# dbking77/ar_slam

Hardware: AMD Instinct MI355X
Metric: LM iterations/sec + ms-to-converged reproj-RMS, 10k-capture synthetic graph (higher is better)
Workload: dtype f64

## Files before the change

ar_slam_amd/build.py:

```python
from __future__ import annotations

import os
import shutil
import subprocess
import sys

HERE = os.path.dirname(os.path.abspath(__file__))
ROOT = os.path.dirname(HERE)
CSRC = os.path.join(HERE, "csrc")
LIB = os.environ.get("ARSLAM_LIB") or os.path.join(HERE, "libarslam_lm.so")
SOURCES = ["lm_kernels.hip", "dense_llt.hip", "lm_solver.hip", "debug_api.hip", "llt_plan.cpp",
           "host_structure.cpp", "localize.hip"]
HOST = os.path.join(HERE, "host")
HOST_SOURCES = ["yaml_lite.cpp", "ar_slam_solver.cpp", "slam_capi.cpp"]
ARCH = os.environ.get("ARSLAM_ARCH", "gfx950")


def hipcc():
    for cand in (shutil.which("hipcc"), "/opt/rocm/bin/hipcc"):
        if cand and os.path.exists(cand):
            return cand
    raise RuntimeError("hipcc not found")


# ... 14 lines not shown
        fcntl.flock(lock, fcntl.LOCK_EX)
        if not force and not _stale():
            return LIB
        return _build_locked(verbose)


def build_id():
    import hashlib
    h = hashlib.sha256(os.environ.get("ARSLAM_EXTRA_FLAGS", "").encode())
    files = [os.path.join(CSRC, f) for f in SOURCES] + [os.path.join(HOST, f) for f in HOST_SOURCES] + \
        sorted(os.path.join(d, f) for d in (CSRC, HOST, os.path.join(ROOT, "include"))
               for f in os.listdir(d) if f.endswith((".h", ".hpp")))
    for f in files:
        with open(f, "rb") as fh:
            h.update(os.path.relpath(f, ROOT).encode() + b"\0" + fh.read())
    commit = "nogit"
    try:
        commit = subprocess.run(["git", "-C", ROOT, "rev-parse", "--short=12", "HEAD"], capture_output=True,
                                text=True, timeout=10).stdout.strip() or "nogit"
        if commit != "nogit":
            rel = [os.path.relpath(f, ROOT) for f in files]
            dirty = subprocess.run(["git", "-C", ROOT, "status", "--porcelain", "--"] + rel, capture_output=True,
                                   text=True, timeout=10).stdout.strip()
            commit += "+dirty" if dirty else ""
    except (OSError, subprocess.SubprocessError):
        pass
    return f"{commit} src {h.hexdigest()[:12]}"


def _build_locked(verbose):
    extra = os.environ.get("ARSLAM_EXTRA_FLAGS", "")
    objdir = os.path.join(HERE, "_obj" + ("_" + "".join(c for c in extra if c.isalnum()) if extra else ""))
    os.makedirs(objdir, exist_ok=True)
    flags = ["-O3", f"--offload-arch={ARCH}", "-fPIC", "-std=c++17", "-munsafe-fp-atomics",
             "-Wall", "-Wno-unused-function", "-I", os.path.join(ROOT, "include"), "-I", CSRC,
             f'-DARSLAM_BUILD_ID="{build_id()}"'] + os.environ.get("ARSLAM_EXTRA_FLAGS", "").split()
    objs = []
    procs = []
    for src in SOURCES:
        obj = os.path.join(objdir, os.path.splitext(src)[0] + ".o")
        cmd = [hipcc()] + flags + (["-x", "hip"] if src.endswith(".cpp") else []) + ["-c", os.path.join(CSRC, src), "-o", obj]
        if verbose:
            print(" ".join(cmd))
        procs.append((src, subprocess.Popen(cmd, stdout=subprocess.PIPE, stderr=subprocess.STDOUT)))
        objs.append(obj)
    for src in HOST_SOURCES:
        obj = os.path.join(objdir, "host_" + os.path.splitext(src)[0] + ".o")
        cmd = ["g++", "-O2", "-fPIC", "-std=c++17", "-Wall", "-I", os.path.join(ROOT, "include"), "-I", CSRC,
               "-I", HOST, "-c", os.path.join(HOST, src), "-o", obj]
        if verbose:
            print(" ".join(cmd))
        procs.append((src, subprocess.Popen(cmd, stdout=subprocess.PIPE, stderr=subprocess.STDOUT)))
        objs.append(obj)
    errs = []
    for src, p in procs:
        out, _ = p.communicate()
        if p.returncode != 0:
            errs.append(f"--- {src} ---\n{out.decode()}")
        elif verbose and out:
            print(out.decode())
    if errs:
        raise RuntimeError("hipcc failed:\n" + "\n".join(errs))
    tmp = f"{LIB}.tmp{os.getpid()}"
    cmd = [hipcc(), f"--offload-arch={ARCH}", "-shared", "-o", tmp] + objs + \
          ["-L/opt/rocm/lib", "-lrccl", "-Wl,-rpath,/opt/rocm/lib"]
    subprocess.check_call(cmd)
    os.replace(tmp, LIB)
# ... 7 lines not shown
```

ar_slam_amd/csrc/debug_api.hip:

```cpp
#include <chrono>
#include "lm_internal.h"
#include "arslam_lm.h"
#include "arslam_lm_debug.h"

#include <climits>
#include <cstdlib>
#include <cstdio>
#include <unistd.h>
#include <cstring>
#include <string>
#include <vector>

namespace arslam {
void debug_read_schur_stamps(unsigned long long *out);
void debug_residual_jacobian(int n, const double *cam, const double *cap, const double *tag,
                             const double *corners, double *r, double *J, hipStream_t s);
void debug_angle_axis(int n, const double *w, const double *p, double *out, int *branch, hipStream_t s);
}

namespace {
int hip_fail(hipError_t e) { return e == hipSuccess ? ARSLAM_OK : ARSLAM_E_HIP; }
}

#define DBG_CHECK(x)                 \
  do {                               \
    hipError_t _e = (x);             \
    if (_e != hipSuccess) return hip_fail(_e); \
  } while (0)

extern "C" int arslam_debug_residual_jacobian(int n, const double *cam, const double *cap,
                                              const double *tag, const double *corners, double *r,
                                              double *J) {
  if (n < 0 || (n && (!cam || !cap || !tag || !corners || !r || !J))) return ARSLAM_E_INVALID_ARG;
  if (n == 0) return ARSLAM_OK;
// ... 373 lines not shown
    return ARSLAM_E_INVALID_ARG;
  }
}

extern "C" int arslam_debug_mixed_groups(const arslam_soa_problem *p, int out[4], unsigned char *e_cap,
                                         unsigned char *e_tag) {
  if (!p || !out) return ARSLAM_E_INVALID_ARG;
  try {
    std::vector<uint8_t> ec, et;
    (void)arslam::ceres_schur_side(p, &ec, &et);
    if (e_cap) std::copy(ec.begin(), ec.end(), e_cap);
    if (e_tag) std::copy(et.begin(), et.end(), e_tag);
    const arslam::MixedProblem m = arslam::mixed_problem(*p, ec, et);
    arslam::HostProblem h = arslam::host_problem(&m.soa, nullptr);
    arslam::mixed_patch(h, m, *p);
    out[0] = h.nc;
    out[1] = h.nt;
    out[2] = m.n_direct;
    out[3] = h.maxblk;
    return ARSLAM_OK;
  } catch (const arslam::ApiError &e) {
    return e.code;
  } catch (...) {
    return ARSLAM_E_INVALID_ARG;
  }
}

extern "C" int arslam_debug_schur_stamps(unsigned long long out[16]) {
  if (!out) return ARSLAM_E_INVALID_ARG;
  arslam::debug_read_schur_stamps(out);
  return ARSLAM_OK;
}

extern "C" int arslam_debug_gather_extend(const arslam_soa_problem *p, int c0, int *identical, int *n_dest) {
  if (!p || !identical || !n_dest || c0 < 0 || c0 > p->n_cap) return ARSLAM_E_INVALID_ARG;
  try {
    std::vector<int> oc, ot;
    std::vector<double> cr;
    for (int b = 0; b < p->n_obs; ++b)
      if (p->obs_cap[b] < c0) {
        oc.push_back(p->obs_cap[b]);
        ot.push_back(p->obs_tag[b]);
        cr.insert(cr.end(), p->corners + 8L * b, p->corners + 8L * b + 8);
      }
    arslam_soa_problem q = *p;
    q.n_cap = c0;
    q.n_obs = (int)oc.size();
    q.obs_cap = oc.data();
    q.obs_tag = ot.data();
    q.corners = cr.data();
    const arslam::HostProblem hs = arslam::host_problem(&q, nullptr);
    const arslam::ReducedLayout L = arslam::reduced_layout(hs, 2, true, nullptr, nullptr);
    arslam::SchurGather G = arslam::schur_gather_plan(hs, L);
    const arslam::HostProblem hf = arslam::host_problem(p, nullptr);
    arslam::schur_gather_extend(G, hf, L, c0);
    const arslam::SchurGather F = arslam::schur_gather_plan(hf, L);
    bool same = G.cap_off == F.cap_off && G.dest_row == F.dest_row && G.dest_start == F.dest_start &&
                G.items == F.items && G.splits == F.splits && G.n_pslots == F.n_pslots &&
                G.max_contrib == F.max_contrib && G.contrib.size() == F.contrib.size();
    for (size_t i = 0; same && i < G.contrib.size(); ++i)
      same = !std::memcmp(&G.contrib[i], &F.contrib[i], sizeof(arslam::SchurContrib));
    *identical = same ? 1 : 0;
    *n_dest = (int)F.dest_start.size() - 1;
    return ARSLAM_OK;
  } catch (const arslam::ApiError &e) {
    return e.code;
// ... 113 lines not shown
```

ar_slam_amd/csrc/host_structure.h:

```cpp
#pragma once

#include "arslam_lm.h"

#include <cstdint>
#include <functional>
#include <stdexcept>
#include <string>
#include <vector>

namespace arslam {

constexpr int kTileRows = 64;
constexpr int kMaxSchurBlocks = 256;

struct ApiError : std::runtime_error {
  int code;
  ApiError(int c, const std::string &m) : std::runtime_error(m), code(c) {}
};

void set_last_error(const std::string &msg);

inline void api_check(bool ok, int code, const char *msg) {
  if (!ok) throw ApiError(code, msg);
}
// ... 57 lines not shown

struct ReducedLayout {
  std::vector<int> tag_row;
  std::vector<int> row_slot;
  int cam_row = -1;
  long nR = 0, N = 0;
  int T = 0;
  std::vector<uint8_t> pattern;
  int n_parts = 0;
  long pad_rows = 0;
  double scalar_flops = 0.0;
  long n_edges = 0;
  long order_edges = 0;
  bool order_reused = false;
};

double scalar_cholesky_flops(const std::vector<std::vector<int>> &adj, const std::vector<int> &tag_row,
                             bool camera);

ReducedLayout reduced_layout(const HostProblem &h, int ordering, bool sparse, const ReduceMaxU8 &adj_max,
                             const ReduceMaxU8 &pattern_max,
                             const std::vector<int> *reuse_tag_row = nullptr, long reuse_edges = 0,
                             bool fast_order = false, bool reuse_by_identity = false);

#if defined(__HIPCC__)
#define ARSLAM_HD __host__ __device__
#else
#define ARSLAM_HD
#endif
struct SchurContrib {
  long off;
  int tr, ld;
};
ARSLAM_HD inline int schur_blk(int x, int m) { return x == 0 ? 0 : (x == m ? 1 + (m - 1) / 6 : 1 + (x - 1) / 6); }
ARSLAM_HD inline int schur_blk_size(int U, int nblk) { return (U == 0 || U == nblk + 1) ? 1 : 6; }
ARSLAM_HD inline int schur_blk_start(int U, int nblk) { return U == 0 ? 0 : (U <= nblk ? 1 + 6 * (U - 1) : 1 + 6 * nblk); }
ARSLAM_HD inline long schur_block_off(int U, int V, int nblk) {
  const long R = U == 0 ? 0 : 1 + 6L * (U - 1) + 18L * U * (U - 1);
  return R + (long)schur_blk_size(U, nblk) * schur_blk_start(V, nblk);
}
ARSLAM_HD inline long schur_slab_size(int nblk) { return 3 + 12L * nblk + 18L * nblk * (nblk + 1); }
constexpr int kSchurChunk = 64;
struct SchurGather {
  std::vector<long> cap_off;
  std::vector<int> dest_row;
  std::vector<int> dest_start;
  std::vector<SchurContrib> contrib;
  std::vector<int> items;
  std::vector<int> splits;
  int n_pslots = 0;
  int max_contrib = 0;
};
SchurGather schur_gather_plan(const HostProblem &h, const ReducedLayout &L);
void schur_gather_extend(SchurGather &G, const HostProblem &h, const ReducedLayout &L, int c0);

}
```

ar_slam_amd/csrc/lm_internal.h:

```cpp
#pragma once
#include <hip/hip_runtime.h>
#include <climits>
#include <cstdint>
#include <stdexcept>
#include <vector>

#include "host_structure.h"

namespace arslam {
constexpr int kCuFlags = 2048;
constexpr int kDagOffTicket0 = 0;
constexpr int kDagOffInflight = 1;
constexpr int kDagOffCuFlags = 2;
constexpr int kDagOffTicket1 = 2 + kCuFlags;
constexpr int kDagOffFault = 3 + kCuFlags;
enum DagFaultField {
  kFaultTicket = 0,
  kFaultKind = 1,
  kFaultCounter = 2,
  kFaultSeen = 3,
  kFaultNeed = 4,
  kFaultDrawn = 5,
  kFaultInflight = 6,
  kFaultBlock = 7,
  kFaultFirstStuck = 8,
  kDagFaultSlots = 9
};
constexpr int kDagOffStarted0 = kDagOffFault + kDagFaultSlots;
constexpr int kDagOffStarted1 = kDagOffStarted0 + 1;
constexpr int kDagCounterExtra = kDagOffStarted1 + 1;
constexpr int kDagWorkgroupsPerCu = 2;

constexpr int kWave = 64;
constexpr int kTile = 64;
constexpr int kRowStride = 14;
constexpr int kJStored = 11;
__host__ __device__ constexpr int jrow_col(int j) {
  return j <= 6 ? j : j <= 9 ? j - 6 : j <= 12 ? j - 3 : 10;
}
constexpr int kObsChunk = 8;
constexpr int kSchurMfmaBlocks = 10;
constexpr size_t schur_lds_bytes(int nblk) {
  return sizeof(double) * (6 * ((6 * nblk + 2) < 64 ? (6 * nblk + 2) : 64) + 6 * kObsChunk + 36 + 36 + 8 +
                           7 * (6 * nblk + 1) + 2 + 28 * nblk) +
         sizeof(int) * (kObsChunk + 2) + 2 * sizeof(double) + 64;
}
static_assert(schur_lds_bytes(kMaxSchurBlocks) <= 160 * 1024, "k_schur's LDS at kMaxSchurBlocks");

enum PartIdx {
  P_COST = 0,
  P_FIXED = 1,
  P_GF = 2,
  P_CF = 3,
  P_MODEL = 4,
  P_STEP2 = 5,
  P_YBAD = 6,
  P_CBAD = 7,
  NPART = 8
};

struct DevProblem {
  int nc, nt, nb;
  long n;
  long nR;
  long N;
  long lda;
  int max_obs_per_cap;
  int max_blk_per_cap;
  const int *big_caps = nullptr;
  int n_big_caps = 0;
  const int *chunk_caps = nullptr;
  int n_chunk_caps = 0;
  int swap_roles;
  const unsigned char *cap_kind = nullptr;
  const int *f_alias = nullptr;
  int nf;
  const int *fslot_row;
  int cam_row;
  const int *cap_start;
  const int *obs_tag;
// ... 266 lines not shown
```

ar_slam_amd/csrc/lm_kernels.hip:

```cpp
#include "lm_internal.h"
#include "projection.h"

#include <cfloat>
#include <mutex>
#include <string>
#include <vector>

#include "arslam_lm.h"
#include <cmath>

namespace arslam {

#ifdef ARSLAM_SCHUR_STAMPS
__device__ unsigned long long g_schur_ph[16];
#define SCHUR_STAMP_INIT unsigned long long _st0 = clock64()
#define SCHUR_STAMP(k)                                                         \
  do {                                                                         \
    const unsigned long long _n = clock64();                                   \
    if (threadIdx.x == 0) atomicAdd(&g_schur_ph[k], _n - _st0);                \
    _st0 = _n;                                                                 \
  } while (0)
void debug_read_schur_stamps(unsigned long long *out) {
  (void)hipMemcpyFromSymbol(out, HIP_SYMBOL(g_schur_ph), sizeof(g_schur_ph));
}
#else
#define SCHUR_STAMP_INIT do {} while (0)
#define SCHUR_STAMP(k) do {} while (0)
void debug_read_schur_stamps(unsigned long long *out) {
  for (int i = 0; i < 16; ++i) out[i] = 0;
}
#endif

namespace {


__device__ __forceinline__ long slot_cap(const DevProblem &P, int c) { return 3 + 6L * c; }
__device__ __forceinline__ long slot_tag(const DevProblem &P, int t) { return 3 + 6L * P.nc + 6L * t; }

__device__ __forceinline__ bool group_swapped(const DevProblem &P, int c) {
  return P.cap_kind ? P.cap_kind[c] == kMixTag : P.swap_roles != 0;
}
__device__ __forceinline__ bool group_direct(const DevProblem &P, int c) {
  return P.cap_kind && P.cap_kind[c] == kMixDirect;
}

__device__ __forceinline__ double lm_d2(const double *diag, long slot, double radius) {
  const double d = sqrt(diag[slot] / radius);
  return d * d;
}

__device__ __forceinline__ void fill_rows(const DevProblem &P, const double *x, const double *scale, int c,
                          int o0, int row0, int nr, int nrows, double *rows, double *gout = nullptr) {
  const double *cam = x;
  const double *cap = x + slot_cap(P, c);
  for (int lr = threadIdx.x; lr < nr; lr += kWave) {
    const int row = row0 + lr;
    const int q = row >> 3, corner = (row >> 1) & 3, comp = row & 1;
    const int obs = o0 + q;
    const int t = P.obs_tag[obs];
    const double *tag = x + slot_tag(P, t);
    double J[13];
    const bool sw = group_swapped(P, c);
    const double r = residual_jacobian_row(cam, sw ? tag : cap, sw ? cap : tag, corner, comp,
                                           P.corners[8L * obs + 2 * corner + comp], J);
    if (sw) {
#pragma unroll
      for (int j = 1; j < 7; ++j) {
// ... 298 lines not shown
        v = kb == 2 ? U[6 * ia + ib] : Etr[ia];
      }
      const int V = schur_blk(q, m), q0V = schur_blk_start(V, nblk);
      dst[(long)sU * q0V + ip * schur_blk_size(V, nblk) + (q - q0V)] = v;
    }
  }
}

template <bool kBig>
__global__ __launch_bounds__(kWave) void k_schur(DevProblem P, const double *__restrict__ scale,
                                                 const double *__restrict__ diag, double radius,
                                                 double *__restrict__ zero_tiles, long n_zero, ExecReset er,
                                                 const int *__restrict__ cap_list) {
  extern __shared__ __attribute__((aligned(16))) double sm[];
  SCHUR_STAMP_INIT;
  const int c = kBig ? cap_list[blockIdx.x] : (int)blockIdx.x, lane = threadIdx.x;
  if (c >= P.nc + n_zero) {
    exec_reset_elem(er, (long)(c - P.nc - n_zero) * kWave + lane);
    return;
  }
  if (c >= P.nc) {
    typedef double d2 __attribute__((ext_vector_type(2)));
    d2 *z = reinterpret_cast<d2 *>(zero_tiles + (long)(c - P.nc) * 4096);
#pragma unroll 8
    for (int e = lane; e < 2048; e += kWave) z[e] = d2{0.0, 0.0};
    return;
  }
  const int o0 = P.cap_start[c], k = P.cap_start[c + 1] - o0;
  if (k == 0) return;
  const int nrows = 8 * k;
  const int b0 = P.cap_blk_start[c], nblk = P.cap_blk_start[c + 1] - b0;
  if (!kBig && nblk > kSchurMfmaBlocks) return;
  const int m = 1 + 6 * nblk;
  double *stage = sm;
  double *tscale = stage + 6 * min(m + 1, kWave);
  double *U = tscale + 6 * kObsChunk;
  double *Ui = U + 36;
  double *Etr = Ui + 36;
  double *W = Etr + 8;
  double *Ftr = W + 6 * m;
  double *FF = Ftr + m + (m & 1);
  int *lblk = (int *)(FF + 28 * nblk);
  double *ff00 = reinterpret_cast<double *>(lblk + kObsChunk);

  const int li = lane & 15, lk = lane >> 4;
  const bool valid = li < 14;
  const double *jb = P.jrows + 8L * o0 * kJStored + (long)jrow_col(min(li, 13)) * nrows;
  double jv[16];
#pragma unroll
  for (int u = 0; u < 8; ++u)
#pragma unroll
    for (int st = 0; st < 2; ++st)
      jv[2 * u + st] = (valid && u < k) ? jb[8 * u + 4 * st + lk] : 0.0;
  static_assert(kObsChunk == 8, "k_schur's operand registers hold eight observations");
  auto stage_chunk = [&](int q0) {
    const int kc = min(kObsChunk, k - q0);
    if (lane < kc) lblk[lane] = P.obs_lblk[o0 + q0 + lane];
    if (lane < 6 * kc) tscale[lane] = scale[slot_tag(P, P.obs_tag[o0 + q0 + lane / 6]) + lane % 6];
  };
  stage_chunk(0);
  __syncthreads();
  SCHUR_STAMP(0);
  {
    for (int e = lane; e < 6 * m + m + (m & 1) + 28 * nblk; e += kWave) W[e] = 0.0;
    __builtin_amdgcn_fence(__ATOMIC_RELEASE, "wavefront");
    __builtin_amdgcn_wave_barrier();
    __builtin_amdgcn_fence(__ATOMIC_ACQUIRE, "wavefront");
    typedef double dbl4v __attribute__((ext_vector_type(4)));
    dbl4v tot = {0, 0, 0, 0};
    const double *sc = scale + slot_cap(P, c);
    const double cs = li == 0 ? scale[0] : li <= 6 ? sc[li - 1] : 1.0;
    const bool tagcol = li >= 7 && li <= 12;
    int acc_off[4], acc_stride[4];
    const int w_base = (int)(W - sm);
    {
      const int c = li, ftr0 = 6 * m, ff0 = ftr0 + m + (m & 1);
// ... 113 lines not shown
        double v = ev[i];
#pragma unroll
        for (int p = i + 1; p < 6; ++p) v -= LI6(p, i) * ev[p];
        ev[i] = v * rd[i];
      }
#pragma unroll
      for (int i = 0; i < 6; ++i) Ui[6 * i + lane] = ev[i];
    }
#undef LI6
  }
  __syncthreads();
  if (lane < 36) P.cap_ui[36L * c + lane] = Ui[lane];
  SCHUR_STAMP(2);
  SCHUR_STAMP(3);
  double *out = P.slab + P.cap_off[c];
  auto make_z = [&](int q, double z[6]) {
    if (q < m) {
      double wq[6];
#pragma unroll
      for (int b = 0; b < 6; ++b) wq[b] = W[b * m + q];
#pragma unroll
      for (int a = 0; a < 6; ++a) {
        double s = 0.0;
#pragma unroll
        for (int b = 0; b < 6; ++b) s += Ui[6 * a + b] * wq[b];
        z[a] = s;
      }
    } else {
#pragma unroll
      for (int a = 0; a < 6; ++a) z[a] = 0.0;
    }
  };
  const bool one_chunk = !kBig;
  double z[6];
  if (one_chunk) make_z(lane, z);
  if (one_chunk) {
    const int M = m + 1;
    const int li = lane & 15, lk = lane >> 4;
    double *Zs = stage;
    if (lane < M)
#pragma unroll
      for (int a = 0; a < 6; ++a) Zs[a * M + lane] = z[a];
    __builtin_amdgcn_fence(__ATOMIC_RELEASE, "wavefront");
    __builtin_amdgcn_wave_barrier();
    __builtin_amdgcn_fence(__ATOMIC_ACQUIRE, "wavefront");
    double Aop[4][2], Bop[4][2];
#pragma unroll
    for (int r = 0; r < 4; ++r)
#pragma unroll
      for (int kb = 0; kb < 2; ++kb) {
        const int a = 4 * kb + lk, pq = 16 * r + li;
        const bool in = a < 6 && pq < M;
        Aop[r][kb] = in ? (pq < m ? W[a * m + pq] : Etr[a]) : 0.0;
        Bop[r][kb] = in ? Zs[a * M + pq] : 0.0;
      }
    typedef double dbl4v __attribute__((ext_vector_type(4)));
#pragma unroll
    for (int r = 0; r < 4; ++r) {
      if (16 * r >= M) break;
      int pU[4], pI[4], pEnd[4];
      long pOff[4];
#pragma unroll
      for (int reg = 0; reg < 4; ++reg) {
        const int pp = 16 * r + lk + 4 * reg;
        const int up = pp >= 1 && pp < m ? (pp - 1) / 6 : -1;
        const int U = pp == 0 ? 0 : (pp < m ? 1 + up : nblk + 1);
        pU[reg] = U;
        pI[reg] = up >= 0 ? pp - 1 - 6 * up : 0;
        pEnd[reg] = pp == 0 ? 1 : (pp < m ? 7 + 6 * up : M);
        pOff[reg] = schur_block_off(U, 0, nblk);
      }
#pragma unroll
      for (int cc = 0; cc < 4; ++cc) {
        if (cc > r + 1 || 16 * cc >= M) break;
        dbl4v acc = {0, 0, 0, 0};
        acc = __builtin_amdgcn_mfma_f64_16x16x4f64(Aop[r][0], Bop[cc][0], acc, 0, 0, 0);
        acc = __builtin_amdgcn_mfma_f64_16x16x4f64(Aop[r][1], Bop[cc][1], acc, 0, 0, 0);
        const int q = 16 * cc + li;
        const int uq = q >= 1 && q < m ? (q - 1) / 6 : -1;
        const int V = q == 0 ? 0 : (q < m ? 1 + uq : nblk + 1);
        const int sV = schur_blk_size(V, nblk), q0V = schur_blk_start(V, nblk);
#pragma unroll
        for (int reg = 0; reg < 4; ++reg) {
          const int pp = 16 * r + lk + 4 * reg;
          if (pp >= M || q >= pEnd[reg]) continue;
          const int U = pU[reg], sU = schur_blk_size(U, nblk);
          double ff = 0.0;
          if (pp == 0) {
            ff = *ff00;
          } else if (pp == m) {
            ff = q < m ? Ftr[q] : 0.0;
          } else {
            const int up = U - 1, i = pI[reg];
            if (q == 0) {
              ff = FF[28 * up + 21 + i];
            } else if (uq == up) {
              const int iq = q - 1 - 6 * uq, lo = min(i, iq), hi = max(i, iq);
              ff = FF[28 * up + lo * 6 - lo * (lo - 1) / 2 + (hi - lo)];
            }
          }
          out[pOff[reg] + (long)sU * q0V + pI[reg] * sV + (q - q0V)] = ff - acc[reg];
        }
      }
    }
  } else
  for (int U = 0; U <= nblk + 1; ++U) {
    const int sU = schur_blk_size(U, nblk), p0U = schur_blk_start(U, nblk), ncol = p0U + sU;
    double *dst = out + schur_block_off(U, 0, nblk);
    for (int q0 = 0; q0 < ncol; q0 += kWave) {
      const int q = q0 + lane;
      if (!one_chunk) make_z(q, z);
      const int V = schur_blk(min(q, m), m), sV = schur_blk_size(V, nblk), q0V = schur_blk_start(V, nblk);
      const int uq = V - 1, iq = q - q0V;
      if (sU == 6) {
        const int up = U - 1;
        double wv[6][6];
#pragma unroll
        for (int i = 0; i < 6; ++i)
#pragma unroll
          for (int a = 0; a < 6; ++a) wv[i][a] = W[a * m + p0U + i];
#pragma unroll
        for (int i = 0; i < 6; ++i) {
          double s = 0.0;
#pragma unroll
          for (int a = 0; a < 6; ++a) s += wv[i][a] * z[a];
          double ff = 0.0;
          if (q == 0) {
            ff = FF[28 * up + 21 + i];
          } else if (uq == up) {
            const int lo = min(i, iq), hi = max(i, iq);
            ff = FF[28 * up + lo * 6 - lo * (lo - 1) / 2 + (hi - lo)];
          }
          if (q < ncol) dst[6 * q0V + i * sV + (q - q0V)] = ff - s;
        }
      } else {
// ... 857 lines not shown
```

ar_slam_amd/lm.py:

```python
from __future__ import annotations

import ctypes as C
import os

import numpy as np

HERE = os.path.dirname(os.path.abspath(__file__))
LIB_PATH = os.environ.get("ARSLAM_LIB") or os.path.join(HERE, "libarslam_lm.so")
MAX_ITERS = 1024
COMM_ID_BYTES = 128

TERMINATION = {0: "CONVERGENCE", 1: "NO_CONVERGENCE", 2: "FAILURE", 3: "USER_SUCCESS", 4: "USER_FAILURE"}
RULES = {0: "none", 1: "gradient_tolerance", 2: "parameter_tolerance", 3: "function_tolerance",
         4: "min_trust_region_radius", 5: "max_num_iterations", 6: "invalid_steps",
         7: "evaluation_failed", 8: "user_callback"}
ERRORS = {-1: "INVALID_ARG", -2: "UNSUPPORTED", -3: "NO_DEVICE", -4: "HIP", -5: "OUT_OF_MEMORY",
          -6: "COMM", -7: "STATE", -8: "DEVICE"}

EXPORTS = ["arslam_lm_options_init", "arslam_lm_create", "arslam_lm_destroy",
           "arslam_lm_set_options", "arslam_lm_get_options",
           "arslam_lm_add_residual_block", "arslam_lm_set_parameter_block_constant",
           "arslam_lm_set_parameter_block_variable", "arslam_lm_solve", "arslam_lm_reset",
           "arslam_lm_num_residual_blocks", "arslam_lm_load_soa", "arslam_lm_solve_loaded",
           "arslam_lm_solve_soa", "arslam_comm_unique_id", "arslam_lm_set_comm", "arslam_lm_set_comm_callback",
           "arslam_device_count", "arslam_lm_last_error", "arslam_lm_version",
           "arslam_lm_set_iteration_callback", "arslam_lm_owned_captures",
           "arslam_debug_residual_jacobian", "arslam_debug_dense_llt", "arslam_debug_dense_llt_ex",
           "arslam_debug_angle_axis_rotate", "arslam_lm_debug_force_indefinite",
           "arslam_lm_debug_force_multirank", "arslam_lm_debug_break_dependency", "arslam_lm_debug_tag_pair_tile",
           "arslam_debug_reduced_plan", "arslam_debug_reduced_plan_side", "arslam_debug_schur_stamps", "arslam_debug_ceres_e_blocks",
           "arslam_debug_mixed_groups",
           "arslam_debug_dag_simulate", "arslam_debug_dag_simulate_started", "arslam_debug_dag_workgroup_limit",
           "arslam_debug_dag_fault_detail", "arslam_debug_box_fingerprint",
           "arslam_debug_rank_split", "arslam_debug_gather_extend",
           "arslam_localize_many", "arslam_localizer_create", "arslam_localizer_destroy",
           "arslam_localizer_load", "arslam_localizer_solve",
           "arslam_slam_create", "arslam_slam_destroy", "arslam_slam_set_verbose", "arslam_slam_load_yaml",
           "arslam_slam_load_yaml_string", "arslam_slam_save_yaml", "arslam_slam_add_detections",
           "arslam_slam_solve", "arslam_slam_solve_incremental", "arslam_slam_localize_many",
           "arslam_slam_num_captures", "arslam_slam_num_arucos", "arslam_slam_num_blocks",
           "arslam_slam_num_solves", "arslam_slam_last_summary", "arslam_slam_solve_summary",
           "arslam_slam_solve_capture", "arslam_slam_unsolved_captures", "arslam_slam_capture", "arslam_slam_set_capture_pose", "arslam_slam_aruco", "arslam_slam_set_aruco_pose",
           "arslam_slam_block", "arslam_slam_camera", "arslam_slam_set_camera",
           "arslam_slam_get_transforms", "arslam_slam_camera_info"]

_dp = C.POINTER(C.c_double)
ALLREDUCE_FN = C.CFUNCTYPE(C.c_int, C.c_void_p, C.c_void_p, C.c_size_t, C.c_int, C.c_int)
SOLVER_CONTINUE, SOLVER_ABORT, SOLVER_TERMINATE_SUCCESSFULLY = 0, 1, 2
ELIM_AUTO, ELIM_CAPTURES, ELIM_TAGS, ELIM_MIXED = 0, 1, 2, 3
SETUP_LOAD, SETUP_VALUES, SETUP_APPEND = 0, 1, 2
_ip = C.POINTER(C.c_int)
_up = C.POINTER(C.c_ubyte)


class LMError(RuntimeError):
    def __init__(self, code, msg):
        super().__init__(f"arslam_lm error {code} ({ERRORS.get(code, '?')}): {msg}")
        self.code = code


class Options(C.Structure):
    _fields_ = [("max_num_iterations", C.c_int),
                ("function_tolerance", C.c_double), ("gradient_tolerance", C.c_double),
                ("parameter_tolerance", C.c_double),
                ("initial_trust_region_radius", C.c_double),
                ("max_trust_region_radius", C.c_double),
                ("min_trust_region_radius", C.c_double),
# ... 112 lines not shown
    L.arslam_localizer_destroy.argtypes = [C.c_void_p]
    L.arslam_localizer_destroy.restype = None
    L.arslam_localizer_load.argtypes = [C.c_void_p, C.POINTER(LocalizeBatchC)]
    L.arslam_localizer_solve.argtypes = [C.c_void_p, _dp, C.POINTER(LocalizeResult), C.POINTER(C.c_double)]
    L.arslam_lm_get_options.argtypes = [C.c_void_p, C.POINTER(Options)]
    L.arslam_lm_destroy.argtypes = [C.c_void_p]
    L.arslam_lm_destroy.restype = None
    L.arslam_lm_add_residual_block.argtypes = [C.c_void_p, _dp, _dp, _dp, _dp]
    L.arslam_lm_set_parameter_block_constant.argtypes = [C.c_void_p, _dp]
    L.arslam_lm_set_parameter_block_variable.argtypes = [C.c_void_p, _dp]
    L.arslam_lm_solve.argtypes = [C.c_void_p, C.POINTER(Summary)]
    L.arslam_lm_reset.argtypes = [C.c_void_p]
    L.arslam_lm_num_residual_blocks.argtypes = [C.c_void_p]
    L.arslam_lm_load_soa.argtypes = [C.c_void_p, C.POINTER(SoaProblem)]
    L.arslam_lm_solve_loaded.argtypes = [C.c_void_p, C.POINTER(Summary)]
    L.arslam_lm_solve_soa.argtypes = [C.POINTER(SoaProblem), C.POINTER(Options), C.POINTER(Summary)]
    L.arslam_comm_unique_id.argtypes = [C.c_char_p]
    L.arslam_lm_set_comm.argtypes = [C.c_void_p, C.c_int, C.c_int, C.c_char_p]
    L.arslam_device_count.argtypes = []
    L.arslam_lm_last_error.restype = C.c_char_p
    L.arslam_lm_version.restype = C.c_char_p
    L.arslam_debug_residual_jacobian.argtypes = [C.c_int, _dp, _dp, _dp, _dp, _dp, _dp]
    L.arslam_debug_dense_llt.argtypes = [C.c_long, _dp, _dp, _dp, C.POINTER(C.c_int)]
    L.arslam_debug_angle_axis_rotate.argtypes = [C.c_int, _dp, _dp, _dp, _ip]
    L.arslam_debug_ceres_e_blocks.argtypes = [C.POINTER(SoaProblem), _ip]
    L.arslam_debug_mixed_groups.argtypes = [C.POINTER(SoaProblem), _ip, C.POINTER(C.c_ubyte), C.POINTER(C.c_ubyte)]
    L.arslam_lm_debug_force_indefinite.argtypes = [C.c_void_p, C.c_ulonglong]
    L.arslam_lm_debug_force_multirank.argtypes = [C.c_void_p, C.c_int]
    L.arslam_debug_dag_workgroup_limit.argtypes = [C.c_int]
    L.arslam_lm_set_iteration_callback.argtypes = [C.c_void_p, ITER_CB, C.c_void_p]
    L.arslam_lm_debug_break_dependency.argtypes = [C.c_void_p, C.c_long, C.POINTER(C.c_long)]
    if hasattr(L, "arslam_lm_debug_tag_pair_tile"):
        L.arslam_lm_debug_tag_pair_tile.argtypes = [C.c_void_p, _dp, _dp, C.POINTER(C.c_int)]
    _lib = L
    return L


def _check(rc):
    if rc != 0:
        raise LMError(rc, lib().arslam_lm_last_error().decode(errors="replace"))


def device_count():
    return lib().arslam_device_count()


def make_options(**kw):
    o = Options()
    lib().arslam_lm_options_init(C.byref(o))
    for k, v in kw.items():
        if not hasattr(o, k):
            raise AttributeError(f"unknown solver option {k}")
        setattr(o, k, v)
    return o


def _f64(a, shape=None):
    a = np.ascontiguousarray(a, dtype=np.float64)
    return a if shape is None else a.reshape(shape)


class _Soa:
    def __init__(self, camera, cap, tag, obs_cap, obs_tag, corners, camera_const=False,
                 cap_const=None, tag_const=None):
        self.camera = _f64(camera).copy()
        self.cap = _f64(cap, (-1, 6)).copy()
# ... 264 lines not shown


def debug_dag_simulate(g, n_workers, seed=1, policy=0, started=None):
    A = _Soa(g.camera, g.cap, g.tag, g.obs_cap, g.obs_tag, g.corners)
    ok = C.c_int(-1)
    if started is None:
        _check(lib().arslam_debug_dag_simulate(C.byref(A.s), int(n_workers), C.c_uint(seed), int(policy),
                                               C.byref(ok)))
    else:
        _check(lib().arslam_debug_dag_simulate_started(C.byref(A.s), int(n_workers), int(started), C.c_uint(seed),
                                                       int(policy), C.byref(ok)))
    return bool(ok.value)


def debug_dag_workgroup_limit(k):
    _check(lib().arslam_debug_dag_workgroup_limit(int(k)))


def debug_dag_fault_detail(g, rec):
    A = _Soa(g.camera, g.cap, g.tag, g.obs_cap, g.obs_tag, g.corners)
    r = (C.c_int * 9)(*([int(v) for v in rec] + [0] * (9 - len(rec))))
    buf = C.create_string_buffer(4096)
    _check(lib().arslam_debug_dag_fault_detail(C.byref(A.s), r, buf, len(buf)))
    return buf.value.decode()


def debug_gather_extend(camera, cap, tag, obs_cap, obs_tag, corners, c0):
    A = _Soa(camera, cap, tag, obs_cap, obs_tag, corners)
    same, nd = C.c_int(0), C.c_int(0)
    _check(lib().arslam_debug_gather_extend(C.byref(A.s), c0, C.byref(same), C.byref(nd)))
    return bool(same.value), nd.value


class SplitInfo(C.Structure):
    _fields_ = [("tiles_per_side", C.c_int), ("n_top_cols", C.c_int), ("n_own_cols", C.c_int),
                ("n_top_tiles", C.c_long), ("n_tiles", C.c_long), ("n_dag_tasks", C.c_long),
                ("phase_split", C.c_long), ("dag_valid", C.c_int), ("n_owned_captures", C.c_int),
                ("top_work", C.c_double), ("max_rank_work", C.c_double), ("total_work", C.c_double),
                ("n_active", C.c_int)]


def debug_rank_split(camera, cap, tag, obs_cap, obs_tag, corners, nranks, rank):
    A = _Soa(camera, cap, tag, obs_cap, obs_tag, corners)
    info = SplitInfo()
    owner = np.zeros(max(A.cap.shape[0], 1), np.int32)
    _check(lib().arslam_debug_rank_split(C.byref(A.s), nranks, rank, C.byref(info), owner.ctypes.data_as(_ip)))
    return {f: getattr(info, f) for f, _ in SplitInfo._fields_}, owner[:A.cap.shape[0]]


def debug_ceres_e_blocks(camera, cap, tag, obs_cap, obs_tag, corners=None, camera_const=False, cap_const=None,
                         tag_const=None):
    if corners is None:
        corners = np.zeros((len(obs_cap), 8))
    A = _Soa(camera, cap, tag, obs_cap, obs_tag, corners, camera_const, cap_const, tag_const)
    out = np.zeros(4, np.int32)
    _check(lib().arslam_debug_ceres_e_blocks(C.byref(A.s), out.ctypes.data_as(_ip)))
    return dict(captures=int(out[0]), tags=int(out[1]), camera=int(out[2]), max_tag_obs=int(out[3]))


def debug_mixed_groups(camera, cap, tag, obs_cap, obs_tag, corners=None, camera_const=False, cap_const=None,
                       tag_const=None):
    if corners is None:
        corners = np.zeros((len(obs_cap), 8))
    A = _Soa(camera, cap, tag, obs_cap, obs_tag, corners, camera_const, cap_const, tag_const)
    out = np.zeros(4, np.int32)
    e_cap = np.zeros(max(A.cap.shape[0], 1), np.uint8)
# ... 237 lines not shown
```

include/arslam_lm_debug.h:

```cpp
#ifndef ARSLAM_LM_DEBUG_H
#define ARSLAM_LM_DEBUG_H

#include "arslam_lm.h"

#ifdef __cplusplus
extern "C" {
#endif

int arslam_debug_residual_jacobian(int n, const double *cam, const double *cap, const double *tag,
                                   const double *corners, double *r, double *J);

int arslam_debug_angle_axis_rotate(int n, const double *w, const double *p, double *out, int *branch);

int arslam_debug_dense_llt(long n, double *A, const double *b, double *y, int *info);
int arslam_debug_dense_llt_ex(long n, double *A, const double *b, double *y, int *info, int executor);

typedef struct {
  long n_reduced;
  long n_padded;
  long pad_rows;
  int tiles_per_side;
  int n_parts;
  int camera_row;
  int n_levels;
// ... 19 lines not shown

int arslam_debug_ceres_e_blocks(const arslam_soa_problem *p, int out[4]);

int arslam_debug_mixed_groups(const arslam_soa_problem *p, int out[4], unsigned char *e_cap, unsigned char *e_tag);

int arslam_debug_reduced_plan(const arslam_soa_problem *p, int ordering, int skip_zero_tiles,
                              arslam_plan_info *info, int *tag_row);
int arslam_debug_reduced_plan_side(const arslam_soa_problem *p, int elimination, arslam_plan_info *info);

int arslam_debug_dag_simulate(const arslam_soa_problem *p, int n_workers, unsigned seed, int policy, int *ok);
int arslam_debug_dag_simulate_started(const arslam_soa_problem *p, int n_workers, int n_started, unsigned seed,
                                      int policy, int *ok);
int arslam_debug_dag_workgroup_limit(int k);

int arslam_debug_dag_fault_detail(const arslam_soa_problem *p, const int rec[9], char *buf, int len);

int arslam_debug_box_fingerprint(int device, double out[6]);

typedef struct {
  int tiles_per_side;
  int n_top_cols;
  int n_own_cols;
  long n_top_tiles;
  long n_tiles;
  long n_dag_tasks, phase_split;
  int dag_valid;
  int n_owned_captures;
  double top_work, max_rank_work, total_work;
  int n_active;
} arslam_split_info;
int arslam_debug_rank_split(const arslam_soa_problem *p, int nranks, int rank, arslam_split_info *info,
                            int *cap_owner);
int arslam_debug_gather_extend(const arslam_soa_problem *p, int c0, int *identical, int *n_dest);

#ifdef __cplusplus
}
#endif
#endif
```

Baseline: 1131.

## Precompute Schur slab store offsets in a constexpr device table

The per-lane index arithmetic in the MFMA Schur store epilogue (block lookup, slab offset, LDS source selection for the FF term) is replaced by a compile-time table. Each entry packs a slab byte offset and an LDS byte offset, with a skip bit. The kernel loads the descriptors as vector words, prefetches the next row tile's descriptors, and writes through raw buffer stores so out-of-range skip entries are dropped by the buffer bounds check. This trades integer ALU and branching for a global-memory table read per lane and longer compile time. It also adds a debug export for checking the table.

```diff
diff --git a/ar_slam_amd/build.py b/ar_slam_amd/build.py
--- a/ar_slam_amd/build.py
+++ b/ar_slam_amd/build.py
@@ -70,7 +70,7 @@
     extra = os.environ.get("ARSLAM_EXTRA_FLAGS", "")
     objdir = os.path.join(HERE, "_obj" + ("_" + "".join(c for c in extra if c.isalnum()) if extra else ""))
     os.makedirs(objdir, exist_ok=True)
-    flags = ["-O3", f"--offload-arch={ARCH}", "-fPIC", "-std=c++17", "-munsafe-fp-atomics",
+    flags = ["-O3", f"--offload-arch={ARCH}", "-fPIC", "-std=c++17", "-munsafe-fp-atomics", "-fconstexpr-steps=100000000",
              "-Wall", "-Wno-unused-function", "-I", os.path.join(ROOT, "include"), "-I", CSRC,
              f'-DARSLAM_BUILD_ID="{build_id()}"'] + os.environ.get("ARSLAM_EXTRA_FLAGS", "").split()
     objs = []
diff --git a/ar_slam_amd/csrc/debug_api.hip b/ar_slam_amd/csrc/debug_api.hip
--- a/ar_slam_amd/csrc/debug_api.hip
+++ b/ar_slam_amd/csrc/debug_api.hip
@@ -1,5 +1,6 @@
 #include <chrono>
 #include "lm_internal.h"
+#include "schur_store_table.h"
 #include "arslam_lm.h"
 #include "arslam_lm_debug.h"
 
@@ -439,6 +440,20 @@
   return ARSLAM_OK;
 }
 
+extern "C" int arslam_debug_schur_store_table(int nblk, int *off, unsigned char *stored) {
+  static constexpr arslam::SchurStoreTable kTable = arslam::make_schur_store_table();
+  if (!off || !stored || nblk < 1 || nblk > arslam::kSchurMfmaBlocks) {
+    arslam::set_last_error("arslam_debug_schur_store_table: nblk outside 1..kSchurMfmaBlocks or a null array");
+    return ARSLAM_E_INVALID_ARG;
+  }
+  const uint32_t *e = &kTable.e[nblk - 1][0][0][0];
+  for (int s = 0; s < arslam::kSchurStoreTiles * arslam::kWave * 4; ++s) {
+    off[s] = (int)((e[s] & arslam::kSchurStoreMask) >> 3);
+    stored[s] = (e[s] >> 31) ? 0 : 1;
+  }
+  return ARSLAM_OK;
+}
+
 extern "C" int arslam_debug_gather_extend(const arslam_soa_problem *p, int c0, int *identical, int *n_dest) {
   if (!p || !identical || !n_dest || c0 < 0 || c0 > p->n_cap) return ARSLAM_E_INVALID_ARG;
   try {
diff --git a/ar_slam_amd/csrc/host_structure.h b/ar_slam_amd/csrc/host_structure.h
--- a/ar_slam_amd/csrc/host_structure.h
+++ b/ar_slam_amd/csrc/host_structure.h
@@ -113,14 +113,14 @@
   long off;
   int tr, ld;
 };
-ARSLAM_HD inline int schur_blk(int x, int m) { return x == 0 ? 0 : (x == m ? 1 + (m - 1) / 6 : 1 + (x - 1) / 6); }
-ARSLAM_HD inline int schur_blk_size(int U, int nblk) { return (U == 0 || U == nblk + 1) ? 1 : 6; }
-ARSLAM_HD inline int schur_blk_start(int U, int nblk) { return U == 0 ? 0 : (U <= nblk ? 1 + 6 * (U - 1) : 1 + 6 * nblk); }
-ARSLAM_HD inline long schur_block_off(int U, int V, int nblk) {
+ARSLAM_HD constexpr int schur_blk(int x, int m) { return x == 0 ? 0 : (x == m ? 1 + (m - 1) / 6 : 1 + (x - 1) / 6); }
+ARSLAM_HD constexpr int schur_blk_size(int U, int nblk) { return (U == 0 || U == nblk + 1) ? 1 : 6; }
+ARSLAM_HD constexpr int schur_blk_start(int U, int nblk) { return U == 0 ? 0 : (U <= nblk ? 1 + 6 * (U - 1) : 1 + 6 * nblk); }
+ARSLAM_HD constexpr long schur_block_off(int U, int V, int nblk) {
   const long R = U == 0 ? 0 : 1 + 6L * (U - 1) + 18L * U * (U - 1);
   return R + (long)schur_blk_size(U, nblk) * schur_blk_start(V, nblk);
 }
-ARSLAM_HD inline long schur_slab_size(int nblk) { return 3 + 12L * nblk + 18L * nblk * (nblk + 1); }
+ARSLAM_HD constexpr long schur_slab_size(int nblk) { return 3 + 12L * nblk + 18L * nblk * (nblk + 1); }
 constexpr int kSchurChunk = 64;
 struct SchurGather {
   std::vector<long> cap_off;
diff --git a/ar_slam_amd/csrc/lm_internal.h b/ar_slam_amd/csrc/lm_internal.h
--- a/ar_slam_amd/csrc/lm_internal.h
+++ b/ar_slam_amd/csrc/lm_internal.h
@@ -46,6 +46,23 @@
          sizeof(int) * (kObsChunk + 2) + 2 * sizeof(double) + 64;
 }
 static_assert(schur_lds_bytes(kMaxSchurBlocks) <= 160 * 1024, "k_schur's LDS at kMaxSchurBlocks");
+struct SchurLds {
+  int tscale, U, Ui, Etr, W, Ftr, FF, lblk, ff00;
+};
+__host__ __device__ constexpr SchurLds schur_lds(int nblk) {
+  const int m = 1 + 6 * nblk;
+  SchurLds l{};
+  l.tscale = 6 * (m + 1 < kWave ? m + 1 : kWave);
+  l.U = l.tscale + 6 * kObsChunk;
+  l.Ui = l.U + 36;
+  l.Etr = l.Ui + 36;
+  l.W = l.Etr + 8;
+  l.Ftr = l.W + 6 * m;
+  l.FF = l.Ftr + m + (m & 1);
+  l.lblk = l.FF + 28 * nblk;
+  l.ff00 = l.lblk + kObsChunk / 2;
+  return l;
+}
 
 enum PartIdx {
   P_COST = 0,
diff --git a/ar_slam_amd/csrc/lm_kernels.hip b/ar_slam_amd/csrc/lm_kernels.hip
--- a/ar_slam_amd/csrc/lm_kernels.hip
+++ b/ar_slam_amd/csrc/lm_kernels.hip
@@ -1,5 +1,6 @@
 #include "lm_internal.h"
 #include "projection.h"
+#include "schur_store_table.h"
 
 #include <cfloat>
 #include <mutex>
@@ -33,6 +34,7 @@
 
 namespace {
 
+__device__ const SchurStoreTable g_schur_store = make_schur_store_table();
 
 __device__ __forceinline__ long slot_cap(const DevProblem &P, int c) { return 3 + 6L * c; }
 __device__ __forceinline__ long slot_tag(const DevProblem &P, int t) { return 3 + 6L * P.nc + 6L * t; }
@@ -397,16 +399,17 @@
   const int b0 = P.cap_blk_start[c], nblk = P.cap_blk_start[c + 1] - b0;
   if (!kBig && nblk > kSchurMfmaBlocks) return;
   const int m = 1 + 6 * nblk;
+  const SchurLds lds = schur_lds(nblk);
   double *stage = sm;
-  double *tscale = stage + 6 * min(m + 1, kWave);
-  double *U = tscale + 6 * kObsChunk;
-  double *Ui = U + 36;
-  double *Etr = Ui + 36;
-  double *W = Etr + 8;
-  double *Ftr = W + 6 * m;
-  double *FF = Ftr + m + (m & 1);
-  int *lblk = (int *)(FF + 28 * nblk);
-  double *ff00 = reinterpret_cast<double *>(lblk + kObsChunk);
+  double *tscale = sm + lds.tscale;
+  double *U = sm + lds.U;
+  double *Ui = sm + lds.Ui;
+  double *Etr = sm + lds.Etr;
+  double *W = sm + lds.W;
+  double *Ftr = sm + lds.Ftr;
+  double *FF = sm + lds.FF;
+  int *lblk = (int *)(sm + lds.lblk);
+  double *ff00 = sm + lds.ff00;
 
   const int li = lane & 15, lk = lane >> 4;
   const bool valid = li < 14;
@@ -586,6 +589,13 @@
     }
   };
   const bool one_chunk = !kBig;
+  typedef unsigned int u4v __attribute__((ext_vector_type(4)));
+  const u4v *desc = reinterpret_cast<const u4v *>(&g_schur_store.e[one_chunk ? nblk - 1 : 0][0][lane][0]);
+  u4v dsc[4];
+  if (one_chunk) {
+    dsc[0] = desc[0];
+    dsc[1] = desc[kWave];
+  }
   double z[6];
   if (one_chunk) make_z(lane, z);
   if (one_chunk) {
@@ -609,20 +619,17 @@
         Bop[r][kb] = in ? Zs[a * M + pq] : 0.0;
       }
     typedef double dbl4v __attribute__((ext_vector_type(4)));
+    typedef unsigned int u2v __attribute__((ext_vector_type(2)));
+    const __amdgpu_buffer_rsrc_t slab_rsrc =
+        __builtin_amdgcn_make_buffer_rsrc(out, 0, (int)(schur_slab_size(nblk) * sizeof(double)), 0x00020000);
 #pragma unroll
     for (int r = 0; r < 4; ++r) {
       if (16 * r >= M) break;
-      int pU[4], pI[4], pEnd[4];
-      long pOff[4];
-#pragma unroll
-      for (int reg = 0; reg < 4; ++reg) {
-        const int pp = 16 * r + lk + 4 * reg;
-        const int up = pp >= 1 && pp < m ? (pp - 1) / 6 : -1;
-        const int U = pp == 0 ? 0 : (pp < m ? 1 + up : nblk + 1);
-        pU[reg] = U;
-        pI[reg] = up >= 0 ? pp - 1 - 6 * up : 0;
-        pEnd[reg] = pp == 0 ? 1 : (pp < m ? 7 + 6 * up : M);
-        pOff[reg] = schur_block_off(U, 0, nblk);
+      u4v dn[4];
+      if (r < 3) {
+#pragma unroll
+        for (int cc = 0; cc < 4; ++cc)
+          if (cc <= r + 2) dn[cc] = desc[(schur_store_row_tile(r + 1) + cc) * kWave];
       }
 #pragma unroll
       for (int cc = 0; cc < 4; ++cc) {
@@ -630,31 +637,20 @@
         dbl4v acc = {0, 0, 0, 0};
         acc = __builtin_amdgcn_mfma_f64_16x16x4f64(Aop[r][0], Bop[cc][0], acc, 0, 0, 0);
         acc = __builtin_amdgcn_mfma_f64_16x16x4f64(Aop[r][1], Bop[cc][1], acc, 0, 0, 0);
-        const int q = 16 * cc + li;
-        const int uq = q >= 1 && q < m ? (q - 1) / 6 : -1;
-        const int V = q == 0 ? 0 : (q < m ? 1 + uq : nblk + 1);
-        const int sV = schur_blk_size(V, nblk), q0V = schur_blk_start(V, nblk);
-#pragma unroll
-        for (int reg = 0; reg < 4; ++reg) {
-          const int pp = 16 * r + lk + 4 * reg;
-          if (pp >= M || q >= pEnd[reg]) continue;
-          const int U = pU[reg], sU = schur_blk_size(U, nblk);
-          double ff = 0.0;
-          if (pp == 0) {
-            ff = *ff00;
-          } else if (pp == m) {
-            ff = q < m ? Ftr[q] : 0.0;
-          } else {
-            const int up = U - 1, i = pI[reg];
-            if (q == 0) {
-              ff = FF[28 * up + 21 + i];
-            } else if (uq == up) {
-              const int iq = q - 1 - 6 * uq, lo = min(i, iq), hi = max(i, iq);
-              ff = FF[28 * up + lo * 6 - lo * (lo - 1) / 2 + (hi - lo)];
-            }
-          }
-          out[pOff[reg] + (long)sU * q0V + pI[reg] * sV + (q - q0V)] = ff - acc[reg];
-        }
+        double ff[4];
+#pragma unroll
+        for (int reg = 0; reg < 4; ++reg)
+          ff[reg] = *reinterpret_cast<const double *>(
+              reinterpret_cast<const char *>(sm) + ((dsc[cc][reg] >> kSchurStoreLdsShift) & kSchurStoreMask));
+#pragma unroll
+        for (int reg = 0; reg < 4; ++reg)
+          __builtin_amdgcn_raw_buffer_store_b64(__builtin_bit_cast(u2v, ff[reg] - acc[reg]), slab_rsrc,
+                                                (int)(dsc[cc][reg] & kSchurStoreMask), 0, 0);
+      }
+      if (r < 3) {
+#pragma unroll
+        for (int cc = 0; cc < 4; ++cc)
+          if (cc <= r + 2) dsc[cc] = dn[cc];
       }
     }
   } else
diff --git a/ar_slam_amd/csrc/schur_store_table.h b/ar_slam_amd/csrc/schur_store_table.h
--- /dev/null
+++ b/ar_slam_amd/csrc/schur_store_table.h
@@ -0,0 +1,57 @@
+#pragma once
+#include <cstdint>
+
+#include "lm_internal.h"
+
+namespace arslam {
+
+constexpr int kSchurStoreTiles = 13;
+constexpr int kSchurStoreLdsShift = 15;
+constexpr uint32_t kSchurStoreMask = 0x7fffu;
+constexpr uint32_t kSchurStoreSkip = 0x80000000u | (kSchurStoreMask & ~7u);
+static_assert(schur_slab_size(kSchurMfmaBlocks) * 8 <= (long)(kSchurStoreMask & ~7u), "slab byte offsets fit 15 bits");
+static_assert(schur_lds(kSchurMfmaBlocks).ff00 * 8 <= (int)kSchurStoreMask, "LDS byte offsets fit 15 bits");
+
+struct alignas(16) SchurStoreTable {
+  uint32_t e[kSchurMfmaBlocks][kSchurStoreTiles][kWave][4];
+};
+__host__ __device__ constexpr int schur_store_row_tile(int r) { return r == 0 ? 0 : r == 1 ? 2 : r == 2 ? 5 : 9; }
+
+constexpr uint32_t schur_store_entry(int nblk, int p, int q) {
+  const int m = 1 + 6 * nblk, M = m + 1;
+  if (p >= M || q >= M) return kSchurStoreSkip;
+  const int U = schur_blk(p, m), V = schur_blk(q, m);
+  if (V > U) return kSchurStoreSkip;
+  const int sV = schur_blk_size(V, nblk);
+  const int i = p - schur_blk_start(U, nblk), j = q - schur_blk_start(V, nblk);
+  const long off = schur_block_off(U, V, nblk) + (long)i * sV + j;
+  const SchurLds l = schur_lds(nblk);
+  int term = l.FF + 27;
+  if (p == 0) {
+    term = l.ff00;
+  } else if (p == m) {
+    if (q < m) term = l.Ftr + q;
+  } else if (q == 0) {
+    term = l.FF + 28 * (U - 1) + 21 + i;
+  } else if (V == U) {
+    const int lo = i < j ? i : j, hi = i < j ? j : i;
+    term = l.FF + 28 * (U - 1) + lo * 6 - lo * (lo - 1) / 2 + (hi - lo);
+  }
+  return (uint32_t)(8 * off) | ((uint32_t)(8 * term) << kSchurStoreLdsShift);
+}
+
+constexpr SchurStoreTable make_schur_store_table() {
+  SchurStoreTable t{};
+  for (int nblk = 1; nblk <= kSchurMfmaBlocks; ++nblk) {
+    int tile = 0;
+    for (int r = 0; r < 4; ++r)
+      for (int cc = 0; cc < 4 && cc <= r + 1; ++cc, ++tile)
+        for (int lane = 0; lane < kWave; ++lane)
+          for (int reg = 0; reg < 4; ++reg)
+            t.e[nblk - 1][tile][lane][reg] =
+                schur_store_entry(nblk, 16 * r + (lane >> 4) + 4 * reg, 16 * cc + (lane & 15));
+  }
+  return t;
+}
+
+}
diff --git a/ar_slam_amd/lm.py b/ar_slam_amd/lm.py
--- a/ar_slam_amd/lm.py
+++ b/ar_slam_amd/lm.py
@@ -32,7 +32,7 @@
            "arslam_debug_mixed_groups",
            "arslam_debug_dag_simulate", "arslam_debug_dag_simulate_started", "arslam_debug_dag_workgroup_limit",
            "arslam_debug_dag_fault_detail", "arslam_debug_box_fingerprint",
-           "arslam_debug_rank_split", "arslam_debug_gather_extend",
+           "arslam_debug_rank_split", "arslam_debug_gather_extend", "arslam_debug_schur_store_table",
            "arslam_localize_many", "arslam_localizer_create", "arslam_localizer_destroy",
            "arslam_localizer_load", "arslam_localizer_solve",
            "arslam_slam_create", "arslam_slam_destroy", "arslam_slam_set_verbose", "arslam_slam_load_yaml",
@@ -211,6 +211,8 @@
     L.arslam_lm_debug_break_dependency.argtypes = [C.c_void_p, C.c_long, C.POINTER(C.c_long)]
     if hasattr(L, "arslam_lm_debug_tag_pair_tile"):
         L.arslam_lm_debug_tag_pair_tile.argtypes = [C.c_void_p, _dp, _dp, C.POINTER(C.c_int)]
+    if hasattr(L, "arslam_debug_schur_store_table"):
+        L.arslam_debug_schur_store_table.argtypes = [C.c_int, _ip, C.POINTER(C.c_ubyte)]
     _lib = L
     return L
 
@@ -541,6 +543,14 @@
     return bool(same.value), nd.value
 
 
+def debug_schur_store_table(nblk):
+    off = np.zeros((13, 64, 4), np.int32)
+    stored = np.zeros((13, 64, 4), np.uint8)
+    _check(lib().arslam_debug_schur_store_table(int(nblk), off.ctypes.data_as(_ip),
+                                                stored.ctypes.data_as(C.POINTER(C.c_ubyte))))
+    return off, stored
+
+
 class SplitInfo(C.Structure):
     _fields_ = [("tiles_per_side", C.c_int), ("n_top_cols", C.c_int), ("n_own_cols", C.c_int),
                 ("n_top_tiles", C.c_long), ("n_tiles", C.c_long), ("n_dag_tasks", C.c_long),
diff --git a/include/arslam_lm_debug.h b/include/arslam_lm_debug.h
--- a/include/arslam_lm_debug.h
+++ b/include/arslam_lm_debug.h
@@ -75,6 +75,7 @@
 int arslam_debug_rank_split(const arslam_soa_problem *p, int nranks, int rank, arslam_split_info *info,
                             int *cap_owner);
 int arslam_debug_gather_extend(const arslam_soa_problem *p, int c0, int *identical, int *n_dest);
+int arslam_debug_schur_store_table(int nblk, int *off, unsigned char *stored);
 
 #ifdef __cplusplus
 }
```

Measured after the change: 1154 (median of 6 runs). +2.1%, better.
